# sashakolpakov/graphem-rapids

Hardware: AMD Instinct MI355X
Metric: layout iterations/s (higher is better)
Workload: dtype f32; 1 GPU; rr1m; graph=rr, n_vertices=1000000, n_edges=4000000, n_components=3, n_neighbors=10, sample_size=256, sampler=device, knn=auto, knn_distance=exact, parallelism=rows/1, reference_identical=False

## Files before the change

### graphem-rapids_amd/csrc/api.hip

```cpp
#include "common.h"
#include "engine.h"
#include "qcell_core.h"

#include "torch_randperm.h"

#include <algorithm>
#include <chrono>
#include <condition_variable>
#include <mutex>
#include <new>
#include <thread>
#include <stdlib.h>
#include <string.h>

static thread_local std::string g_create_error;
void gh_set_create_error(const std::string &msg) { g_create_error = msg; }

gh_scope::gh_scope(gh_engine *h_, const char *name, hipStream_t on) : h(h_), stream(on ? on : h_->stream) {
    if (!h->timing) return;
    for (size_t i = 0; i < h->timers.size(); ++i)
        if (h->timers[i].name == name) slot = (int)i;
    if (slot < 0) {
        h->timers.emplace_back();
        h->timers.back().name = name;
// ... 74 lines not shown
    sw.no_presetup = getenv("GRAPHEM_HIP_NO_PRESETUP") != nullptr;
    sw.reorder = getenv("GRAPHEM_HIP_REORDER");
    if (const char *e = getenv("GRAPHEM_HIP_TAU_SEPARATE")) sw.tau_separate = atoi(e) != 0;
    sw.stamps = getenv("GRAPHEM_HIP_STAMPS") != nullptr;
    return sw;
}

static gh_status allocate_and_upload(gh_engine *h, const gh_graph_plan &g, const create_switches &sw) {
    const int64_t n = h->n, E = h->E;
    const int D = h->D;
    const bool hashed = h->part.edge_rule == GH_EDGES_HASHED;
    const size_t nLD = (size_t)n * h->LD, S = (size_t)h->S;
    gh_status st;
#define GH_A(p, count, zero) GH_TRY_ST(gh_alloc(h, h->p, (count), (zero)))
    GH_A(d_edges, (size_t)E * 2, false);
    GH_A(d_rowptr, (size_t)h->rows + 1, false);
    GH_A(d_adj, (size_t)h->adj_len, false);
    GH_A(d_first_edge, (size_t)h->rows + 1, true);
    GH_A(d_mid, (size_t)h->own_count * h->LD, true);
    GH_A(d_Fs, (size_t)h->rows * h->LD, true);
    const bool scan_path = gh_knn_scan_path(h);
    GH_A(d_gmin, (size_t)gh_gmin_floats(h), true);
    GH_A(d_sub_uv, (size_t)h->thr_M1 * 2, false);
    if (hashed) GH_A(d_own_eids, g.own_eids.size() + 1, true);
    if (h->nlong) {
        GH_A(d_long_rows, g.long_rows.size(), false);
        GH_A(d_long_ownptr, g.long_ownptr.size(), false);
        GH_A(d_long_ownadj, g.long_ownadj.size() + 1, true);
        GH_A(d_long_eptr, g.long_eptr.size(), false);
        GH_A(d_long_erow, g.long_erow.size() + 1, false);
        GH_A(d_long_terms, (size_t)h->long_entries * D, false);
        GH_A(d_own_long, g.own_long.size(), false);
    }
    GH_A(d_vblock, g.vblock.size(), false);
    GH_A(d_pos, (size_t)h->pos_rows * h->LD, true);
    GH_A(d_new_buf, (size_t)h->rows * h->LD, true);
    h->d_new = h->d_new_buf.p;
    GH_A(d_tmpF, nLD, true);
    GH_A(d_tmpF2, nLD, true);
    GH_A(d_io, (size_t)n * D, false);
    GH_A(d_acc, nLD, true);
    GH_A(d_tflag, (size_t)n, true);
    GH_A(d_touched, 4 * S * (size_t)h->k, false);
    GH_A(d_tcount, 1, true);
    GH_A(d_sampled, S, true);
    GH_A(d_q, S * (size_t)(h->LD + 4), true);
// ... 244 lines not shown
    }
    if (gh_grid_path(h)) {
        GH_TRY_ST(gh_knn_prepare(h));
        GH_TRY_ST(gh_launch_spring_mid(h));
        GH_TRY_ST(gh_grid_search(h));
        return gh_knn_finish(h, true, fuse_intersect);
    }
    if (gh_ivf_path(h)) {
        GH_TRY_ST(gh_knn_prepare(h));
        GH_TRY_ST(gh_launch_spring_mid(h));
        GH_TRY_ST(gh_ivf_search(h));
        return gh_knn_finish(h, true, fuse_intersect);
    }
    if (h->fused_scan && gh_knn_scan_path(h)) {
        GH_TRY_ST(gh_knn_prepare(h));
        if (!h->tau_embedded) GH_TRY_ST(gh_knn_thresholds(h));
        GH_TRY_ST(gh_launch_spring_scan(h));
        return gh_knn_finish(h, false, fuse_intersect);
    }
    GH_TRY_ST(gh_launch_spring_mid(h));
    return gh_knn_local(h, fuse_intersect);
}

static gh_status step_merge(gh_engine *h, const uint64_t *gathered, int world) {
    GH_TRY_ST(gh_knn_merge(h, gathered, world));
    if (!h->intersect_done) GH_TRY_ST(gh_launch_intersect(h));
    GH_TRY_ST(gh_launch_integrate(h));
    return GH_OK;
}

static gh_status step_finish(gh_engine *h, const gh_ids *next) {
    const bool presetup = next && h->rows == h->n && h->layout != GH_LAYOUT_GATHERED && gh_knn_scan_path(h) &&
                          (h->fused_scan || gh_grid_path(h) || gh_ivf_path(h)) && h->S > 0 && h->k > 0 && !h->opt_no_presetup;
    GH_TRY_ST(gh_launch_normalise(h, true, presetup ? next : nullptr));
    h->iter += 1;
    return GH_OK;
}

template <class Src, class Before>
static gh_status run_iterations(gh_engine *h, int32_t iters, bool draws_own, Src src_of_row, Before before_row) {
    const gh_ids own = gh_own_ids(h);
    auto loop = [&]() -> gh_status {
        for (int32_t t = 0; t < iters; ++t) {
            GH_TRY_ST(before_row(t));
            h->sample = src_of_row(t);
            GH_TRY_ST(step_begin(h, true));
            GH_TRY_ST(step_merge(h, h->d_partial.p, 1));
            const gh_ids next = t + 1 < iters ? src_of_row(t + 1) : own;
            GH_TRY_ST(step_finish(h, t + 1 < iters || draws_own ? &next : nullptr));
        }
        return GH_OK;
    };
    const gh_status st = loop();
    h->sample = gh_ids{GH_IDS_GIVEN, h->d_sampled.p};
    return st;
}
static gh_status nothing_before(int32_t) { return GH_OK; }

extern "C" gh_status gh_step(gh_handle h, const int32_t *sampled) {
    GH_TRY_ST(check_handle(h));
    if (h->f64) return gh_f64_step(h, sampled);
    GH_TRY_ST(check_whole(h, "gh_step"));
    GH_TRY_ST(check_k(h));
    gh_ids src;
    GH_TRY_ST(caller_ids(h, sampled, &src));
    return run_iterations(h, 1, sampled == nullptr, [&](int32_t) { return src; }, nothing_before);
}

static gh_status ensure_stream_ids(gh_engine *h, size_t words) {
    if (words <= h->stream_ids_cap) return GH_OK;
    if (h->d_stream_ids.p) { GH_HIP(hipStreamSynchronize(h->stream)); h->d_stream_ids.reset(); h->stream_ids_cap = 0; }
    GH_TRY_ST(gh_alloc(h, h->d_stream_ids, words, false));
// ... 571 lines not shown
```

### graphem-rapids_amd/csrc/engine.h

```cpp
#pragma once
#include <hip/hip_runtime.h>
#include <stdint.h>
#include <memory>
#include <string>
#include <vector>

#include "../../include/graphem_hip.h"
#include "host_util.h"

#define GH_CAND_CAP 16384
#define GH_SEL_BUF 4096
#define GH_SEL_CHUNK 2048
#define GH_CNT_STRIDE 32
#define GH_POS_PAD_ROWS 1024
inline int gh_fix_blocks(int LD) { return LD <= 16 ? 2 * LD : 0; }
#define GH_SCAN_MIN_EDGES 16384

struct gh_timer_slot {
    std::string name;
    double total_ms = 0.0;
    int64_t launches = 0;
    std::vector<std::pair<hipEvent_t, hipEvent_t>> pending;
};

// ... 83 lines not shown
    float *d_new = nullptr;
    gh_dev<float> d_tmpF;
    gh_dev<float> d_tmpF2;
    gh_dev<float> d_io;

    gh_dev<double> d_acc;
    gh_dev<int32_t> d_tflag;
    gh_dev<int32_t> d_touched;
    gh_dev<int32_t> d_tcount;

    gh_dev<int32_t> d_sampled;
    gh_ids sample{};
    gh_dev<int32_t> d_stream_ids;
    size_t stream_ids_cap = 0;
    gh_ring ring;
    double sampler_stats[4] = {0, 0, 0, 0};
    bool new0_ready = false;
    bool intersect_done = false;
    bool stats_reduced = false;
    struct {
        bool valid = false;
        gh_ids src{};
        uint64_t iter = 0;
    } lookahead;
    bool last_step_own_ids = false;
    bool tcount_reset_pending = false;
    gh_dev<float> d_iscratch;
    gh_dev<float> d_q;
    gh_dev<float> d_qscan;
    gh_dev<uint16_t> d_qA;
    gh_dev<int32_t> d_order;
    std::vector<int32_t> order_host;
    gh_dev<unsigned char> d_gbuf;
    int64_t g_slot = 0, g_chunk = 0;
    int g_world = 0, g_rank = 0;
    int layout = GH_LAYOUT_NONE;
    gh_dev<float> d_rows_packed;
    bool packed_exchange = false;
    bool rows_early = false;
    gh_dev<float> d_rows_all;
    gh_dev<float> d_rows_pk;
    gh_dev<double> d_stats_all;
    int64_t stats_block = 0;
    int64_t patch_cap = 0;
    gh_dev<int32_t> d_qexact;
    gh_dev<uint64_t> d_cand;
    gh_dev<int32_t> d_cnt;
// ... 41 lines not shown
#define GH_STAMP_EXTRA 8192
    gh_dev<unsigned long long> d_stamps;
    bool timing = false;
    std::vector<gh_timer_slot> timers;

    std::unique_ptr<gh_ivf, gh_part_delete> ivf;
    std::unique_ptr<gh_f64, gh_part_delete> f64;
    std::unique_ptr<gh_comm, gh_part_delete> comm;
};

template <class T> gh_status gh_alloc(gh_engine *h, gh_dev<T> &buf, size_t count, bool zero) {
    if (count == 0) count = 1;
    if (!buf.alloc(count * sizeof(T))) {
        h->err = std::string("hipMalloc failed: ") + hipGetErrorString(hipGetLastError());
        return GH_ERR_NOMEM;
    }
    if (zero) GH_HIP(hipMemsetAsync(buf.p, 0, count * sizeof(T), h->stream));
    return GH_OK;
}

inline gh_ids gh_own_ids(const gh_engine *h) { return gh_ids{h->S >= h->E ? GH_IDS_ARANGE : GH_IDS_SAMPLER, h->d_sampled.p}; }
inline void gh_set_lookahead(gh_engine *h, const gh_ids *next) {
    h->lookahead.valid = next != nullptr;
    if (next) { h->lookahead.src = *next; h->lookahead.iter = h->iter + 1; }
}

struct gh_scope {
    gh_engine *h;
    int slot = -1;
    hipEvent_t a = nullptr, b = nullptr;
    hipStream_t stream = nullptr;
    gh_scope(gh_engine *h_, const char *name, hipStream_t on = nullptr );
    ~gh_scope();
};

struct gh_graph_plan {
    const int32_t *edges = nullptr;
    std::vector<int32_t> internal;
    std::vector<int32_t> rowptr, adj;
    std::vector<int32_t> first_edge, own_eids, vblock;
    std::vector<int32_t> long_rows, long_ownptr, long_ownadj, long_eptr, long_erow;
    std::vector<uint8_t> own_long;
    std::vector<int32_t> sub_uv;
};
void gh_plan_graph(gh_engine *h, const int32_t *edges, bool partitioned, int reorder, gh_graph_plan *g);
void gh_auto_knn_method(gh_engine *h);
void gh_plan_threshold_subset(const gh_engine *h, gh_graph_plan *g);
// ... 27 lines not shown
gh_status gh_knn_points_device(hipStream_t stream, const float *d_q, int64_t nq, const float *d_ref, int64_t nref,
                               int D, int K, uint64_t *d_keys, std::string *err);
gh_status gh_cdist_alloc(gh_engine *h);
gh_status gh_knn_merge_cdist(gh_engine *h, const uint64_t *gathered, int world);
gh_status gh_knn_finish_cdist(gh_engine *h, bool all_rows, bool fuse_intersect);
bool gh_grid_path(const gh_engine *h);
gh_status gh_grid_alloc(gh_engine *h);
gh_status gh_grid_search(gh_engine *h);
bool gh_ivf_path(const gh_engine *h);
gh_status gh_ivf_alloc(gh_engine *h);
gh_status gh_ivf_search(gh_engine *h);
gh_status gh_radial_topk_device(gh_engine *h, int K, uint64_t *d_part, int nparts, int32_t *d_ids);
int gh_fused_mfma_kb(const gh_engine *h);
bool gh_fused_uses_mfma(const gh_engine *h);
int gh_fused_tile(const gh_engine *h);
bool gh_fused_cells_ok(const gh_engine *h);
void gh_choose_scan_filter(gh_engine *h);
gh_status gh_launch_spring_scan(gh_engine *h);
gh_status gh_knn_merge(gh_engine *h, const uint64_t *gathered, int world);
gh_status gh_launch_intersect(gh_engine *h);
gh_status gh_launch_inter_cleanup(gh_engine *h);
gh_status gh_launch_spring_mid(gh_engine *h);
gh_status gh_launch_mid_only(gh_engine *h);
gh_status gh_launch_integrate(gh_engine *h);
gh_status gh_launch_spring_only(gh_engine *h, float *d_F);
gh_status gh_launch_inter_to_dense(gh_engine *h, float *d_F);
gh_status gh_launch_integrate_given(gh_engine *h, const float *d_Fs, const float *d_Fi);
gh_status gh_launch_normalise(gh_engine *h, bool with_cleanup, const gh_ids *next = nullptr, bool gathered = false,
                              const double *stats_all = nullptr);
gh_status gh_launch_unpack_rows(gh_engine *h);
struct gh_long_args;
gh_long_args gh_make_long_args(const gh_engine *h, bool coop_mid = false);
gh_status gh_launch_spring_long(gh_engine *h, float *outF, int64_t f_row0);
inline int32_t *gh_patch_count(gh_engine *h) { return reinterpret_cast<int32_t *>(h->d_stats + (size_t)(2 + 2 * gh_fix_blocks(h->LD)) * h->LD); }
inline float *gh_patch_records(gh_engine *h) { return reinterpret_cast<float *>(gh_patch_count(h) + 4); }
gh_status gh_launch_new0(gh_engine *h);
gh_status gh_launch_pack_rows(gh_engine *h, hipStream_t stream);
gh_status gh_launch_patch_rows(gh_engine *h);
gh_status gh_launch_pad(gh_engine *h, const float *d_src_nD, float *d_dst_nLD);
gh_status gh_launch_unpad(gh_engine *h, const float *d_src_nLD, float *d_dst_nD);
gh_status gh_launch_sample(gh_engine *h);
gh_status gh_launch_arange(gh_engine *h);
gh_status gh_ensure_sample(gh_engine *h);
```

### graphem-rapids_amd/csrc/forces.hip

```cpp
#include "common.h"
#include "engine.h"
#include "intersect_core.h"
#include "setup_core.h"

namespace {

template <int D, int LD, bool WRITE_MID, bool LONG>
__global__ __launch_bounds__(256) void spring_kernel(
    const float *__restrict__ pos, const int32_t *__restrict__ rowptr, const int32_t *__restrict__ adj,
    const int32_t *__restrict__ first_edge, int64_t edge_lo, int64_t row_lo, int64_t rows, float L_min,
    float neg_k, float *__restrict__ outF, int64_t f_row0, float *__restrict__ mid, gh_long_args la) {
    const int64_t i = blockIdx.x * (int64_t)blockDim.x + threadIdx.x;
    if (i >= rows) return;
    const int64_t x = row_lo + i;
    float px[LD], F[LD];
    gh_load_row<LD>(pos, x, px);
    int64_t mid_row0 = 0;
    if (WRITE_MID) mid_row0 = first_edge[i] - edge_lo;
    if constexpr (LONG)
        spring_row<D, LD, WRITE_MID>(pos, adj, rowptr[i], rowptr[i + 1], x, px, L_min, neg_k, F, mid, mid_row0, la, (int)i,
                                     outF + (i + f_row0) * LD);
    else
        spring_pull<D, LD, WRITE_MID>(pos, adj, rowptr[i], rowptr[i + 1], x, px, L_min, neg_k, F, mid, mid_row0);
    gh_store_row<LD>(outF, i + f_row0, F);
// ... 194 lines not shown
}

__global__ __launch_bounds__(256) void stats_reduce_kernel(const double *__restrict__ blockstats, int nblocks, int LD,
                                                          double *__restrict__ stats) {
    const int c = blockIdx.x;
    double s = 0.0;
    for (int b = threadIdx.x; b < nblocks; b += blockDim.x) s += blockstats[(int64_t)c * nblocks + b];
    __shared__ double red[4];
    const double a = gh_wave_sum(s);
    if ((threadIdx.x & 63) == 0) red[threadIdx.x >> 6] = a;
    __syncthreads();
    if (threadIdx.x == 0) stats[c] = ((red[0] + red[1]) + red[2]) + red[3];
}

template <int LD>
__global__ __launch_bounds__(256) void stats_fix_kernel(const double *__restrict__ blockstats, int nblocks,
                                                       const float *__restrict__ pos, const float *__restrict__ Fs,
                                                       const double *__restrict__ acc,
                                                       const int32_t *__restrict__ touched,
                                                       const int32_t *__restrict__ tcount, int64_t row_lo,
                                                       int64_t rows, float *__restrict__ out_new,
                                                       double *__restrict__ stats, int skip_reduce,
                                                       int32_t *__restrict__ patch_count = nullptr ,
                                                       float *__restrict__ patch_rows = nullptr, int patch_cap = 0) {
    __shared__ double red[4][2 * LD];
    const int lane = threadIdx.x & 63, w = threadIdx.x >> 6;
    if (!skip_reduce) {
        const int c = blockIdx.x;
        double s = 0.0;
        double s4[4] = {0.0, 0.0, 0.0, 0.0};
        const double *col = blockstats + (int64_t)c * nblocks;
        int b = threadIdx.x;
        for (; b + 3 * (int)blockDim.x < nblocks; b += 4 * blockDim.x) {
#pragma unroll
            for (int u = 0; u < 4; ++u) s4[u] += col[b + u * blockDim.x];
        }
        for (int u = 0; b < nblocks; b += blockDim.x, ++u) s4[u] += col[b];
        s = (s4[0] + s4[1]) + (s4[2] + s4[3]);
        const double a = gh_wave_sum(s);
        if (lane == 0) red[w][0] = a;
        __syncthreads();
        if (threadIdx.x == 0) stats[c] = ((red[0][0] + red[1][0]) + red[2][0]) + red[3][0];
        __syncthreads();
    }
    double dx[LD], dxx[LD];
#pragma unroll
    for (int d = 0; d < LD; ++d) { dx[d] = 0.0; dxx[d] = 0.0; }
    const int nt = *tcount;
    for (int t = blockIdx.x * blockDim.x + threadIdx.x; t < nt; t += gridDim.x * blockDim.x) {
        const int64_t x = touched[t];
        const int64_t i = x - row_lo;
        if (i < 0 || i >= rows) continue;
        float p[LD], f[LD], nw[LD];
        gh_load_row<LD>(pos, x, p);
        gh_load_row<LD>(Fs, i, f);
#pragma unroll
        for (int d = 0; d < LD; ++d) {
            const float n0 = p[d] + f[d];
            const float tot = f[d] + (float)acc[x * LD + d];
            nw[d] = p[d] + tot;
            dx[d] += (double)nw[d] - (double)n0;
            dxx[d] += (double)nw[d] * (double)nw[d] - (double)n0 * (double)n0;
        }
        if (!patch_count) gh_store_row<LD>(out_new, i, nw);
        else gh_patch_append<LD>(patch_count, patch_rows, patch_cap, x, nw);
    }
#pragma unroll
    for (int d = 0; d < LD; ++d) {
        const double a = gh_wave_sum(dx[d]), b = gh_wave_sum(dxx[d]);
        if (lane == 0) { red[w][d] = a; red[w][LD + d] = b; }
    }
    __syncthreads();
// ... 10 lines not shown
        const int64_t x = touched[t / LD];
        const int d = (int)(t % LD);
        acc[x * LD + d] = 0.0;
        if (d == 0) tflag[x] = 0;
    }
}

struct gh_norm_src {
    const float *rows;
    int64_t chunk;
    int64_t block;
    int RS;
    int64_t out_lo, out_rows;
    const double *stats;
    int world;
    int64_t stats_block;
    __device__ const float *row(int64_t j) const {
        const float *p = rows;
        for (; j >= chunk; j -= chunk) p += block;
        return p + j * RS;
    }
};

template <int LDT>
__global__ __launch_bounds__(256) void normalise_kernel(gh_norm_src src, int D, int LD, int64_t n, float *__restrict__ pos,
                                                       double *__restrict__ acc ,
                                                       int32_t *__restrict__ tflag,
                                                       const int32_t *__restrict__ touched,
                                                       const int32_t *__restrict__ tcount, int nfix, int g_norm,
                                                       int n_setup, gh_setup_args sa, int32_t *__restrict__ qexact,
                                                       unsigned long long *__restrict__ stamps ,
                                                       float *__restrict__ packed = nullptr ) {
    if (stamps && (blockIdx.x >= GH_STAMP_EXTRA)) stamps = nullptr;
    if (stamps) stamps += (int64_t)blockIdx.x * 8;
#define GH_STAMP(k) do { if (stamps && threadIdx.x == 0) stamps[k] = wall_clock64(); } while (0)
    GH_STAMP(0);
    __shared__ __align__(16) unsigned char setup_lds[GH_SETUP_LDS_BYTES];
    const bool setup_block = (int)blockIdx.x < n_setup;
    const int nb = (int)blockIdx.x - n_setup;
    if (acc && !setup_block)
        gh_clear_touched(acc, tflag, touched, tcount, LD, nb * (int64_t)blockDim.x + threadIdx.x, (int64_t)g_norm * blockDim.x);
    constexpr int LDS_ = LDT > 0 ? LDT : 4;
    constexpr bool early_fetch = LDT > 0 && LDT <= 8;
    gh_setup_rows<LDS_> srows;
    auto raw_row = [=](int64_t v, float (&row)[LDS_]) {
        const float *p = src.row(v);
        if (src.RS == LD) {
            gh_load_row<LDS_>(p, 0, row);
        } else {
#pragma unroll
            for (int d = 0; d < LDS_; ++d) row[d] = d < D ? p[d] : 0.0f;
        }
    };
    if constexpr (early_fetch)
        if (setup_block && sa.tiles > 0) gh_setup_fetch<LDS_>(sa, (int)blockIdx.x, raw_row, srows);
    extern __shared__ float ms[];
    double *srow = reinterpret_cast<double *>(ms + 2 * LD);
    const int R = 2 + 2 * nfix;
    double *tot = srow + R * LD;
    for (int r = 0; r < src.world; ++r) {
        const double *st = src.stats + (int64_t)r * src.stats_block;
        for (int t = threadIdx.x; t < R * LD; t += blockDim.x) srow[t] = st[t];
        __syncthreads();
        for (int d = threadIdx.x; d < LD; d += blockDim.x) {
            double sum = srow[d], sq = srow[LD + d];
#pragma unroll 8
            for (int b = 0; b < nfix; ++b) {
                sum += srow[(2 + 2 * b) * LD + d];
                sq += srow[(3 + 2 * b) * LD + d];
            }
            sum = (r > 0 ? tot[d] : 0.0) + sum;
            sq = (r > 0 ? tot[LD + d] : 0.0) + sq;
            if (r + 1 < src.world) {
                tot[d] = sum;
                tot[LD + d] = sq;
                continue;
            }
            float mean = 0.0f, sd = 1.0f;
            if (d < D) {
                const double m = sum / (double)n;
                double var = (sq - sum * m) / (double)(n - 1);
                if (var < 0.0) var = 0.0;
                mean = (float)m;
                sd = (float)sqrt(var) + 1e-6f;
            }
            ms[d] = mean;
            ms[LD + d] = sd;
        }
        __syncthreads();
    }
    GH_STAMP(1);
    if (stamps && threadIdx.x == 0) stamps[6] = setup_block ? 1 : 2;
    if (setup_block) {
        const int64_t t = (int64_t)blockIdx.x * blockDim.x + threadIdx.x;
        if (t == 0) qexact[0] = 0;
        auto getp = [=](int64_t v, int d) { return (src.row(v)[d] - ms[d]) / ms[LD + d]; };
        if constexpr (LDT > 0) {
            if (sa.tiles > 0) {
                auto norm = [=](float x, int d) { return (x - ms[d]) / ms[LD + d]; };
                if constexpr (!early_fetch) gh_setup_fetch<LDS_>(sa, (int)blockIdx.x, raw_row, srows);
                gh_setup_finish<LDS_>(sa, (int)blockIdx.x, raw_row, norm, srows, setup_lds, stamps);
            } else {
                gh_setup_item(sa, t, getp);
            }
        } else {
            gh_setup_item(sa, t, getp);
        }
        GH_STAMP(3);
        return;
    }
    const int64_t step = (int64_t)g_norm * blockDim.x;
    const float *in = src.rows;
    for (int64_t j0 = 0; j0 < src.out_rows; j0 += src.chunk, in += src.block) {
        const int64_t total4 = min(src.chunk, src.out_rows - j0) * LD / 4;
        float4 *dst = reinterpret_cast<float4 *>(pos + (src.out_lo + j0) * LD);
        auto norm4 = [&](int64_t t, const float4 &v) {
            const int d0 = (int)((t * 4) % LD);
            float4 o;
            o.x = d0 + 0 < D ? (v.x - ms[d0 + 0]) / ms[LD + d0 + 0] : 0.0f;
            o.y = d0 + 1 < D ? (v.y - ms[d0 + 1]) / ms[LD + d0 + 1] : 0.0f;
            o.z = d0 + 2 < D ? (v.z - ms[d0 + 2]) / ms[LD + d0 + 2] : 0.0f;
            o.w = d0 + 3 < D ? (v.w - ms[d0 + 3]) / ms[LD + d0 + 3] : 0.0f;
            dst[t] = o;
            if (packed) {
// ... 253 lines not shown
    if (M == 0) return GH_OK;
    gh_scope t(h, "mid_gather");
    mid_gather_kernel<<<dim3(grid_for(M * h->LD, 256)), dim3(256), 0, h->stream>>>(
        h->d_pos.p, h->d_edges.p, h->part.edge_lo, h->d_own_eids.p, M, h->D, h->LD, h->d_mid.p);
    GH_LAUNCH_CHECK();
    return GH_OK;
}

}

gh_status gh_launch_spring_mid(gh_engine *h) {
    const bool fused = h->fused_mid && gh_dim_templated(h->D);
    if (h->rows > 0) {
        gh_scope t(h, fused ? "spring_mid" : "spring");
        gh_status st = fused ? launch_spring<true>(h, h->d_Fs.p, 0) : launch_spring<false>(h, h->d_Fs.p, 0);
        if (st) return st;
    }
    if (!fused) return launch_mid_gather(h);
    return GH_OK;
}

gh_status gh_launch_mid_only(gh_engine *h) { return launch_mid_gather(h); }

gh_status gh_launch_integrate(gh_engine *h) {
    if (h->new0_ready && h->rows > 0) {
        h->new0_ready = false;
        gh_scope t(h, "stats_fix");
        const struct reset_flag { gh_engine *e; ~reset_flag() { e->stats_reduced = false; } } reset{h};
        if (!gh_dispatch_stride(h->LD, [&](auto ld) {
                stats_fix_kernel<ld()><<<dim3(gh_fix_blocks(ld())), dim3(256), 0, h->stream>>>(
                    h->d_blockstats.p, h->n_vblocks, h->d_pos.p, h->d_Fs.p, h->d_acc.p, h->d_touched.p, h->d_tcount.p, h->part.row_lo,
                    h->rows, h->d_new, h->d_stats, h->stats_reduced ? 1 : 0,
                    h->layout == GH_LAYOUT_OVERLAP ? gh_patch_count(h) + (h->iter & 1) : nullptr,
                    h->layout == GH_LAYOUT_OVERLAP ? gh_patch_records(h) : nullptr, (int)h->patch_cap);
            })) {
            h->err = "stats_fix: the fused step left its sums for a row stride other than 4, 8 or 16";
            return GH_ERR_RUNTIME;
        }
        GH_LAUNCH_CHECK();
        return GH_OK;
    }
    h->new0_ready = false;
    GH_HIP(hipMemsetAsync(h->d_stats + 2 * h->LD, 0, sizeof(double) * 2 * gh_fix_blocks(h->LD) * h->LD, h->stream));
    if (h->rows == 0) {
        GH_HIP(hipMemsetAsync(h->d_stats, 0, sizeof(double) * 2 * h->LD, h->stream));
        return GH_OK;
    }
    const unsigned grid = grid_for(h->rows, 256);
    int32_t *pc = h->layout == GH_LAYOUT_OVERLAP ? gh_patch_count(h) + (h->iter & 1) : nullptr;
    float *pr = h->layout == GH_LAYOUT_OVERLAP ? gh_patch_records(h) : nullptr;
    const int pcap = (int)h->patch_cap;
    float *wide_out = h->d_new;
    {
        gh_scope t(h, "integrate");
        if (!gh_dispatch_stride(h->LD, [&](auto ld) {
                integrate_kernel<ld()><<<dim3(grid), dim3(256), 0, h->stream>>>(h->d_pos.p, h->d_Fs.p, h->part.row_lo, h->rows, h->d_acc.p,
                                                                               h->d_tflag.p, h->d_new, h->d_blockstats.p, pc, pr, pcap);
            }))
            integrate_generic_kernel<<<dim3(grid_for(h->rows * h->LD, 256)), dim3(256), 0, h->stream>>>(
                h->d_pos.p, h->d_Fs.p, h->LD, h->part.row_lo, h->rows, h->d_acc.p, h->d_tflag.p, wide_out);
        GH_LAUNCH_CHECK();
    }
// ... 43 lines not shown

gh_status gh_launch_inter_cleanup(gh_engine *h) {
    const int64_t maxT = 4 * h->S * h->k * h->LD;
    if (maxT == 0) return GH_OK;
    gh_scope t(h, "inter_cleanup");
    inter_cleanup_kernel<<<dim3(grid_for(maxT, 256)), dim3(256), 0, h->stream>>>(h->d_acc.p, h->d_tflag.p, h->d_touched.p,
                                                                                 h->d_tcount.p, h->LD);
    reset_counter_kernel<<<dim3(1), dim3(1), 0, h->stream>>>(h->d_tcount.p);
    GH_LAUNCH_CHECK();
    return GH_OK;
}

gh_status gh_launch_integrate_given(gh_engine *h, const float *d_Fs, const float *d_Fi) {
    GH_HIP(hipMemsetAsync(h->d_stats, 0, sizeof(double) * (2 + 2 * gh_fix_blocks(h->LD)) * h->LD, h->stream));
    const int64_t total = h->n * h->LD;
    integrate_given_kernel<<<dim3(grid_for(total, 256)), dim3(256), 0, h->stream>>>(h->d_pos.p, d_Fs, d_Fi, total,
                                                                                    h->d_new);
    column_stats_kernel<<<dim3(h->D), dim3(256), 0, h->stream>>>(h->d_new, h->n, h->D, h->LD, h->d_stats);
    GH_LAUNCH_CHECK();
    return GH_OK;
}

gh_status gh_launch_normalise(gh_engine *h, bool with_cleanup, const gh_ids *next, bool gathered, const double *stats_all) {
    gh_set_lookahead(h, nullptr);
    const int R = 2 + 2 * gh_fix_blocks(h->LD);
    gh_norm_src src{h->d_new, std::max<int64_t>(h->rows, 1), 0, h->LD, h->part.row_lo, h->rows, h->d_stats, 1, 0};
    if (stats_all) {
        src.stats = stats_all;
        src.world = h->g_world;
        src.stats_block = (int64_t)R * h->LD;
    }
    if (gathered) {
        const bool overlap = h->layout == GH_LAYOUT_OVERLAP;
        src.RS = overlap && h->d_rows_pk.p ? h->D : h->LD;
        src.rows = overlap ? (h->d_rows_pk.p ? h->d_rows_pk.p : h->d_rows_all.p) : reinterpret_cast<const float *>(h->d_gbuf.p);
        src.chunk = std::min(h->g_chunk, h->n);
        src.block = overlap ? h->g_chunk * src.RS : h->g_slot / (int64_t)sizeof(float);
        src.out_lo = 0;
        src.out_rows = h->n;
        src.stats = overlap ? h->d_stats_all.p : reinterpret_cast<const double *>(h->d_gbuf.p + h->g_chunk * h->LD * (int64_t)sizeof(float));
        src.world = h->g_world;
        src.stats_block = overlap ? h->stats_block : h->g_slot / (int64_t)sizeof(double);
        if (!(h->fused_scan && gh_knn_scan_path(h) && h->S > 0 && h->k > 0 && !h->opt_no_presetup)) next = nullptr;
    }
    if (src.out_rows == 0) return with_cleanup ? gh_launch_inter_cleanup(h) : GH_OK;
    gh_scope t(h, gathered ? "normalise_gathered" : stats_all ? "normalise_own" : "normalise");
    unsigned grid = grid_for(src.out_rows * h->LD / 4, 1024);
    if (grid > 2048) grid = 2048;
    gh_setup_args sa{};
    unsigned extra = 0;
    if (next) {
        sa = gh_make_setup_args(h, *next, h->iter + 1);
        extra = gh_setup_blocks(sa);
    }
    const size_t smem = sizeof(float) * 2 * h->LD + sizeof(double) * (size_t)(R + (src.world > 1 ? 2 : 0)) * h->LD;
    float *packed = stats_all && h->packed_exchange ? h->d_rows_packed.p + (size_t)h->g_rank * h->g_chunk * h->D : nullptr;
    const int ldt = stats_all ? 0 : h->LD;
    const auto normalise = [&](auto ld) {
        normalise_kernel<ld()><<<dim3(grid + extra), dim3(256), smem, h->stream>>>(
            src, h->D, h->LD, h->n, h->d_pos.p, with_cleanup ? h->d_acc.p : nullptr, h->d_tflag.p, h->d_touched.p, h->d_tcount.p,
            gh_fix_blocks(h->LD), (int)grid, (int)extra, sa, h->d_qexact.p,
            h->d_stamps.p ? h->d_stamps.p + (int64_t)std::max(h->n_vblocks, 1) * 8 : nullptr, packed);
    };
    if (!gh_dispatch_stride(ldt, normalise)) {
        if (sa.tiles > 0) { h->err = "KNN set-up tiles need a row stride of 4, 8 or 16"; return GH_ERR_RUNTIME; }
        normalise(gh_int<0>{});
    }
    GH_LAUNCH_CHECK();
    gh_set_lookahead(h, next);
    return GH_OK;
}

__global__ __launch_bounds__(256) void unpack_rows_kernel(const float *__restrict__ packed, int64_t n, int D, int LD, int64_t own_lo,
                                                         int64_t own_hi, float *__restrict__ pos) {
    const int64_t t = blockIdx.x * (int64_t)256 + threadIdx.x;
    if (t >= n * LD) return;
    const int64_t row = t / LD;
    const int d = (int)(t % LD);
    if (row >= own_lo && row < own_hi) return;
    pos[t] = d < D ? packed[row * D + d] : 0.0f;
}
gh_status gh_launch_unpack_rows(gh_engine *h) {
    if (!h->packed_exchange) return GH_OK;
    gh_scope t(h, "unpack_rows");
    unpack_rows_kernel<<<dim3(grid_for(h->n * h->LD, 256)), dim3(256), 0, h->stream>>>(h->d_rows_packed.p, h->n, h->D, h->LD, h->part.row_lo,
// ... 111 lines not shown
```

### graphem-rapids_amd/csrc/knn.hip

```cpp
#include "common.h"
#include "engine.h"
#include "scan_core.h"
#include "setup_core.h"
#include "tau_core.h"
#include "intersect_core.h"
#include "select_core.h"

#include <math.h>
#include <type_traits>
#include <stdlib.h>

namespace {


__global__ __launch_bounds__(256) void knn_setup_kernel(const float *__restrict__ pos, gh_setup_args a,
                                                       int32_t *__restrict__ tcount, int32_t *__restrict__ qexact) {
    __shared__ __align__(16) unsigned char lds[GH_SETUP_LDS_BYTES];
    if (blockIdx.x == 0 && threadIdx.x == 0) { *tcount = 0; qexact[0] = 0; }
    const int LD = a.LD;
    auto getp = [=](int64_t v, int d) { return pos[v * LD + d]; };
    if (a.tiles > 0) gh_setup_block_any(a, (int)blockIdx.x, getp, lds);
    else gh_setup_item(a, blockIdx.x * (int64_t)blockDim.x + threadIdx.x, getp);
}

// ... 439 lines not shown
    return GH_OK;
}

}

static int64_t own_edges(const gh_engine *h) { return h->own_count; }

bool gh_knn_scan_path(const gh_engine *h) {
    const int64_t Mtot = own_edges(h);
    return Mtot >= GH_SCAN_MIN_EDGES && h->LD <= 16 && h->D >= 2 && h->Ksel <= GH_EXTRACT_MAX_K && h->S <= 0x7FFFFFFF;
}

void gh_choose_threshold_subset(gh_engine *h) {
    const int64_t Mtot = own_edges(h);
    const bool scan = gh_knn_scan_path(h) && !gh_grid_path(h) && !gh_ivf_path(h);
    h->thr_stride = scan ? subset_stride(Mtot, h->Ksel, h->S, gh_fused_tile(h), gh_fused_uses_mfma(h)) : 1;
    h->thr_M1 = scan ? (Mtot + h->thr_stride - 1) / h->thr_stride : 0;
}

gh_setup_args gh_make_setup_args(const gh_engine *h, gh_ids src, uint64_t iter) {
    const int tiles = (int)((h->thr_M1 + GH_THR_TILE - 1) / GH_THR_TILE);
    return gh_setup_args{h->d_edges.p, src.ids, src.mode, h->E, h->prm.seed, iter, h->S, h->D, h->LD, h->d_q.p, h->d_cnt.p,
                         h->d_ovf.p, h->part.edge_lo, h->d_own_eids.p, reinterpret_cast<const int2 *>(h->d_sub_uv.p), h->thr_M1, h->thr_stride, h->d_gmin.p,
                         (int64_t)tiles * GH_THR_GROUPS, tiles, h->tau_embedded ? h->d_tau_flag.p : nullptr};
}

unsigned gh_setup_blocks(const gh_setup_args &a) {
    return a.tiles > 0 ? (unsigned)a.tiles : (unsigned)((a.S + 255) / 256);
}
int64_t gh_gmin_floats(const gh_engine *h) {
    const gh_setup_args a = gh_make_setup_args(h, gh_ids{GH_IDS_GIVEN, nullptr}, 0);
    if (gh_ivf_path(h)) return h->S * 256 + 4;
    if (a.tiles == 0) return 4;
    return h->S * a.Gpad + 4;
}

gh_status gh_knn_prepare(gh_engine *h) {
    const gh_ids src = h->sample;
    h->sample.mode = GH_IDS_GIVEN;
    const bool done = h->lookahead.valid && h->lookahead.iter == h->iter && h->lookahead.src.mode == src.mode &&
                      h->lookahead.src.ids == src.ids;
    gh_set_lookahead(h, nullptr);
    h->tcount_reset_pending = done;
    if (done) return GH_OK;
    const gh_setup_args a = gh_make_setup_args(h, src, h->iter);
    gh_scope t(h, "knn_setup");
    knn_setup_kernel<<<dim3(gh_setup_blocks(a)), dim3(256), 0, h->stream>>>(h->d_pos.p, a, h->d_tcount.p, h->d_qexact.p);
// ... 178 lines not shown
```

### graphem-rapids_amd/csrc/setup_core.h

```cpp
#pragma once
#include "common.h"
#include "engine.h"
#include "scan_core.h"

struct gh_setup_args {
    const int32_t *edges;
    int32_t *sampled;
    int mode;
    int64_t E;
    uint64_t seed, iter;
    int64_t S;
    int D, LD;
    float *qt;
    int32_t *cnt, *ovf;
    int64_t e_lo;
    const int32_t *own_eids;
    const int2 *sub_uv;
    int64_t M1, stride;
    float *gmin;
    int64_t Gpad;
    int tiles;
    unsigned *tau_flag;
};

#define GH_THR_TILE 128
#define GH_THR_GSIZE 64
#define GH_THR_GROUPS (GH_THR_TILE / GH_THR_GSIZE)

template <class P >
__device__ __forceinline__ void gh_setup_item(const gh_setup_args &a, int64_t t, P getp) {
    if (t == 0 && a.tau_flag) *a.tau_flag = 0;
    if (t >= a.S) return;
    int32_t e32;
    if (a.mode == 1) { e32 = gh_sample_id(a.E, a.seed, a.iter, t); a.sampled[t] = e32; }
    else if (a.mode == 2) { e32 = (int32_t)t; a.sampled[t] = e32; }
    else e32 = a.sampled[t];
    const int QS = gh_qs(a.D, a.LD);
    const int64_t e = e32;
    const int64_t u = a.edges[2 * e], v = a.edges[2 * e + 1];
    for (int d = 0; d < QS; ++d) a.qt[t * QS + d] = d < a.D ? (getp(u, d) + getp(v, d)) / 2.0f : 0.0f;
    a.qt[t * QS + gh_qtau(a.D, a.LD)] = INFINITY;
    a.cnt[t * GH_CNT_STRIDE] = 0;
    a.ovf[t] = 0;
}

template <int CTRL>
__device__ __forceinline__ uint32_t gh_dpp_u32(uint32_t v) {
    return (uint32_t)__builtin_amdgcn_update_dpp((int)v, (int)v, CTRL, 0xF, 0xF, false);
}
__device__ __forceinline__ uint32_t gh_row_min_u32(uint32_t v) {
    v = min(v, gh_dpp_u32<0xB1>(v));
    v = min(v, gh_dpp_u32<0x4E>(v));
    v = min(v, gh_dpp_u32<0x141>(v));
    v = min(v, gh_dpp_u32<0x140>(v));
    return v;
}

#define GH_SETUP_LDS_BYTES (GH_THR_TILE * 16 * 4)
template <int LD>
struct gh_setup_rows {
    float qa[LD], qb[LD], ma[LD], mb[LD];
    int32_t e32;
};
template <int LD, class RAW >
__device__ __forceinline__ void gh_setup_fetch(const gh_setup_args &a, int blk, RAW raw, gh_setup_rows<LD> &st) {
    const int t = threadIdx.x;
    __builtin_amdgcn_s_setprio(3);
    if (blk == 0 && t == 0 && a.tau_flag) *a.tau_flag = 0;
    st.e32 = 0;
#pragma unroll
    for (int d = 0; d < LD; ++d) { st.qa[d] = 0.0f; st.qb[d] = 0.0f; st.ma[d] = 0.0f; st.mb[d] = 0.0f; }
    if (t < a.S) {
        if (a.mode == 1) st.e32 = gh_sample_id(a.E, a.seed, a.iter, t);
        else if (a.mode == 2) st.e32 = (int32_t)t;
        else st.e32 = a.sampled[t];
        const int2 uv = reinterpret_cast<const int2 *>(a.edges)[st.e32];
        raw(uv.x, st.qa);
        raw(uv.y, st.qb);
    }
    if (t < GH_THR_TILE) {
        const int64_t j = (int64_t)blk * GH_THR_TILE + t;
        if (j < a.M1) {
            const int2 uv = a.sub_uv[j];
            raw(uv.x, st.ma);
            raw(uv.y, st.mb);
        }
    }
}

template <int LD, class RAW, class NORM >
__device__ __forceinline__ void gh_setup_finish(const gh_setup_args &a, int blk, RAW raw, NORM norm, const gh_setup_rows<LD> &st,
                                                unsigned char *lds, unsigned long long *stamps = nullptr ) {
    gh_f2 *rsh = reinterpret_cast<gh_f2 *>(lds);
    const int t = threadIdx.x;
    auto query = [&](int64_t s, int32_t &e32, float (&q)[LD]) {
        if (a.mode == 1) e32 = gh_sample_id(a.E, a.seed, a.iter, s);
        else if (a.mode == 2) e32 = (int32_t)s;
        else e32 = a.sampled[s];
        const int2 uv = reinterpret_cast<const int2 *>(a.edges)[e32];
        float ra[LD], rb[LD];
        raw(uv.x, ra);
        raw(uv.y, rb);
#pragma unroll
        for (int d = 0; d < LD; ++d) q[d] = d < a.D ? (norm(ra[d], d) + norm(rb[d], d)) / 2.0f : 0.0f;
    };
    float q[LD];
    int32_t e32 = st.e32;
#pragma unroll
    for (int d = 0; d < LD; ++d) q[d] = d < a.D ? (norm(st.qa[d], d) + norm(st.qb[d], d)) / 2.0f : 0.0f;
    if (t < GH_THR_TILE) {
        const int64_t j = (int64_t)blk * GH_THR_TILE + t;
        float m[LD];
#pragma unroll
        for (int d = 0; d < LD; ++d) m[d] = 0.0f;
        if (j < a.M1) {
#pragma unroll
            for (int d = 0; d < LD; ++d)
                if (d < a.D) m[d] = (norm(st.ma[d], d) + norm(st.mb[d], d)) / 2.0f;
        } else {
            m[0] = INFINITY;
        }
        float *slot = reinterpret_cast<float *>(rsh + (t >> 1) * LD) + (t & 1);
#pragma unroll
        for (int d = 0; d < LD; ++d) slot[2 * d] = m[d];
    }
// ... 36 lines not shown
            }
            mn[gg] = best;
        }
        static_assert(GH_THR_GROUPS == 2 || GH_THR_GROUPS % 4 == 0, "vector stores of the group minima");
        if constexpr (GH_THR_GROUPS == 2) {
            *reinterpret_cast<uint2 *>(dst) = make_uint2(mn[0], mn[1]);
        } else {
#pragma unroll
            for (int g4 = 0; g4 < GH_THR_GROUPS; g4 += 4)
                *reinterpret_cast<uint4 *>(dst + g4) = make_uint4(mn[g4], mn[g4 + 1], mn[g4 + 2], mn[g4 + 3]);
        }
    }
}

template <int LD, class P>
__device__ __forceinline__ void gh_setup_block(const gh_setup_args &a, int blk, P getp, unsigned char *lds,
                                               unsigned long long *stamps = nullptr ) {
    auto raw = [&](int64_t v, float (&row)[LD]) {
#pragma unroll
        for (int d = 0; d < LD; ++d) row[d] = d < a.D ? getp(v, d) : 0.0f;
    };
    auto norm = [](float x, int) { return x; };
    gh_setup_rows<LD> st;
    gh_setup_fetch<LD>(a, blk, raw, st);
    gh_setup_finish<LD>(a, blk, raw, norm, st, lds, stamps);
}

template <class P>
__device__ __forceinline__ void gh_setup_block_any(const gh_setup_args &a, int blk, P getp, unsigned char *lds,
                                                   unsigned long long *stamps = nullptr) {
    if (a.LD == 4) gh_setup_block<4>(a, blk, getp, lds, stamps);
    else if (a.LD == 8) gh_setup_block<8>(a, blk, getp, lds, stamps);
    else gh_setup_block<16>(a, blk, getp, lds, stamps);
}
```

Baseline: 6496 iterations/s.

## Stage next-iteration KNN setup endpoint rows during stats_fix kernel

The stats_fix launch gains extra blocks that gather the next iteration's sampled edge endpoint rows (new position computed from pos, Fs and acc, or taken from new0) into a staging buffer. The normalise kernel's KNN setup tiles can then read those contiguous rows instead of doing random edge and position lookups. This moves scattered gather latency into a kernel that was lightly occupied and removes repeated per-tile random reads. It adds a buffer, a lookahead validity flag and a second template instantiation, and it depends on the staged rows matching what normalise would have computed.

```diff
diff --git a/graphem-rapids_amd/csrc/api.hip b/graphem-rapids_amd/csrc/api.hip
--- a/graphem-rapids_amd/csrc/api.hip
+++ b/graphem-rapids_amd/csrc/api.hip
@@ -120,6 +120,7 @@
     const bool scan_path = gh_knn_scan_path(h);
     GH_A(d_gmin, (size_t)gh_gmin_floats(h), true);
     GH_A(d_sub_uv, (size_t)h->thr_M1 * 2, false);
+    if (h->thr_M1 > 0 && h->rows == n) GH_A(d_setup_rows, 2 * S * h->LD, true);
     if (hashed) GH_A(d_own_eids, g.own_eids.size() + 1, true);
     if (h->nlong) {
         GH_A(d_long_rows, g.long_rows.size(), false);
@@ -410,17 +411,20 @@
     return gh_knn_local(h, fuse_intersect);
 }
 
-static gh_status step_merge(gh_engine *h, const uint64_t *gathered, int world) {
+static gh_status step_merge(gh_engine *h, const uint64_t *gathered, int world, const gh_ids *next = nullptr) {
     GH_TRY_ST(gh_knn_merge(h, gathered, world));
     if (!h->intersect_done) GH_TRY_ST(gh_launch_intersect(h));
-    GH_TRY_ST(gh_launch_integrate(h));
-    return GH_OK;
-}
-
-static gh_status step_finish(gh_engine *h, const gh_ids *next) {
+    GH_TRY_ST(gh_launch_integrate(h, next));
+    return GH_OK;
+}
+
+static const gh_ids *presetup_ids(const gh_engine *h, const gh_ids *next) {
     const bool presetup = next && h->rows == h->n && h->layout != GH_LAYOUT_GATHERED && gh_knn_scan_path(h) &&
                           (h->fused_scan || gh_grid_path(h) || gh_ivf_path(h)) && h->S > 0 && h->k > 0 && !h->opt_no_presetup;
-    GH_TRY_ST(gh_launch_normalise(h, true, presetup ? next : nullptr));
+    return presetup ? next : nullptr;
+}
+static gh_status step_finish(gh_engine *h, const gh_ids *next) {
+    GH_TRY_ST(gh_launch_normalise(h, true, presetup_ids(h, next)));
     h->iter += 1;
     return GH_OK;
 }
@@ -433,9 +437,10 @@
             GH_TRY_ST(before_row(t));
             h->sample = src_of_row(t);
             GH_TRY_ST(step_begin(h, true));
-            GH_TRY_ST(step_merge(h, h->d_partial.p, 1));
             const gh_ids next = t + 1 < iters ? src_of_row(t + 1) : own;
-            GH_TRY_ST(step_finish(h, t + 1 < iters || draws_own ? &next : nullptr));
+            const gh_ids *next_ids = t + 1 < iters || draws_own ? &next : nullptr;
+            GH_TRY_ST(step_merge(h, h->d_partial.p, 1, presetup_ids(h, next_ids)));
+            GH_TRY_ST(step_finish(h, next_ids));
         }
         return GH_OK;
     };
diff --git a/graphem-rapids_amd/csrc/engine.h b/graphem-rapids_amd/csrc/engine.h
--- a/graphem-rapids_amd/csrc/engine.h
+++ b/graphem-rapids_amd/csrc/engine.h
@@ -129,7 +129,9 @@
         bool valid = false;
         gh_ids src{};
         uint64_t iter = 0;
+        bool rows = false;
     } lookahead;
+    gh_dev<float> d_setup_rows;
     bool last_step_own_ids = false;
     bool tcount_reset_pending = false;
     gh_dev<float> d_iscratch;
@@ -217,7 +219,18 @@
 inline gh_ids gh_own_ids(const gh_engine *h) { return gh_ids{h->S >= h->E ? GH_IDS_ARANGE : GH_IDS_SAMPLER, h->d_sampled.p}; }
 inline void gh_set_lookahead(gh_engine *h, const gh_ids *next) {
     h->lookahead.valid = next != nullptr;
+    h->lookahead.rows = false;
     if (next) { h->lookahead.src = *next; h->lookahead.iter = h->iter + 1; }
+}
+inline void gh_set_lookahead_rows(gh_engine *h, const gh_ids &next) {
+    h->lookahead.valid = false;
+    h->lookahead.rows = true;
+    h->lookahead.src = next;
+    h->lookahead.iter = h->iter + 1;
+}
+inline bool gh_lookahead_rows_for(const gh_engine *h, const gh_ids *next) {
+    return next && h->lookahead.rows && h->lookahead.iter == h->iter + 1 && h->lookahead.src.mode == next->mode &&
+           h->lookahead.src.ids == next->ids;
 }
 
 struct gh_scope {
@@ -291,7 +304,7 @@
 gh_status gh_launch_inter_cleanup(gh_engine *h);
 gh_status gh_launch_spring_mid(gh_engine *h);
 gh_status gh_launch_mid_only(gh_engine *h);
-gh_status gh_launch_integrate(gh_engine *h);
+gh_status gh_launch_integrate(gh_engine *h, const gh_ids *next = nullptr);
 gh_status gh_launch_spring_only(gh_engine *h, float *d_F);
 gh_status gh_launch_inter_to_dense(gh_engine *h, float *d_F);
 gh_status gh_launch_integrate_given(gh_engine *h, const float *d_Fs, const float *d_Fi);
diff --git a/graphem-rapids_amd/csrc/forces.hip b/graphem-rapids_amd/csrc/forces.hip
--- a/graphem-rapids_amd/csrc/forces.hip
+++ b/graphem-rapids_amd/csrc/forces.hip
@@ -240,7 +240,14 @@
                                                        int64_t rows, float *__restrict__ out_new,
                                                        double *__restrict__ stats, int skip_reduce,
                                                        int32_t *__restrict__ patch_count = nullptr ,
-                                                       float *__restrict__ patch_rows = nullptr, int patch_cap = 0) {
+                                                       float *__restrict__ patch_rows = nullptr, int patch_cap = 0,
+                                                       gh_setup_args sa = gh_setup_args{} ,
+                                                       const int32_t *__restrict__ tflag = nullptr, float *__restrict__ setup_rows = nullptr) {
+    constexpr int NFIX = 2 * LD;
+    if ((int)blockIdx.x >= NFIX) {
+        gh_setup_gather<LD>(sa, gh_gather_src{pos, Fs, out_new, acc, tflag, setup_rows}, (int)blockIdx.x - NFIX);
+        return;
+    }
     __shared__ double red[4][2 * LD];
     const int lane = threadIdx.x & 63, w = threadIdx.x >> 6;
     if (!skip_reduce) {
@@ -265,7 +272,7 @@
 #pragma unroll
     for (int d = 0; d < LD; ++d) { dx[d] = 0.0; dxx[d] = 0.0; }
     const int nt = *tcount;
-    for (int t = blockIdx.x * blockDim.x + threadIdx.x; t < nt; t += gridDim.x * blockDim.x) {
+    for (int t = blockIdx.x * blockDim.x + threadIdx.x; t < nt; t += NFIX * blockDim.x) {
         const int64_t x = touched[t];
         const int64_t i = x - row_lo;
         if (i < 0 || i >= rows) continue;
@@ -322,7 +329,7 @@
     }
 };
 
-template <int LDT>
+template <int LDT, bool STAGED>
 __global__ __launch_bounds__(256) void normalise_kernel(gh_norm_src src, int D, int LD, int64_t n, float *__restrict__ pos,
                                                        double *__restrict__ acc ,
                                                        int32_t *__restrict__ tflag,
@@ -353,7 +360,7 @@
         }
     };
     if constexpr (early_fetch)
-        if (setup_block && sa.tiles > 0) gh_setup_fetch<LDS_>(sa, (int)blockIdx.x, raw_row, srows);
+        if (setup_block && sa.tiles > 0) gh_setup_fetch<LDS_, STAGED>(sa, (int)blockIdx.x, raw_row, srows);
     extern __shared__ float ms[];
     double *srow = reinterpret_cast<double *>(ms + 2 * LD);
     const int R = 2 + 2 * nfix;
@@ -398,8 +405,8 @@
         if constexpr (LDT > 0) {
             if (sa.tiles > 0) {
                 auto norm = [=](float x, int d) { return (x - ms[d]) / ms[LD + d]; };
-                if constexpr (!early_fetch) gh_setup_fetch<LDS_>(sa, (int)blockIdx.x, raw_row, srows);
-                gh_setup_finish<LDS_>(sa, (int)blockIdx.x, raw_row, norm, srows, setup_lds, stamps);
+                if constexpr (!early_fetch) gh_setup_fetch<LDS_, STAGED>(sa, (int)blockIdx.x, raw_row, srows);
+                gh_setup_finish<LDS_, STAGED>(sa, (int)blockIdx.x, raw_row, norm, srows, setup_lds, stamps);
             } else {
                 gh_setup_item(sa, t, getp);
             }
@@ -699,22 +706,31 @@
 
 gh_status gh_launch_mid_only(gh_engine *h) { return launch_mid_gather(h); }
 
-gh_status gh_launch_integrate(gh_engine *h) {
+gh_status gh_launch_integrate(gh_engine *h, const gh_ids *next) {
+    h->lookahead.rows = false;
     if (h->new0_ready && h->rows > 0) {
         h->new0_ready = false;
         gh_scope t(h, "stats_fix");
         const struct reset_flag { gh_engine *e; ~reset_flag() { e->stats_reduced = false; } } reset{h};
+        gh_setup_args sa{};
+        unsigned gather = 0;
+        if (next && h->d_setup_rows.p && h->rows == h->n && h->part.row_lo == 0 && h->layout == GH_LAYOUT_NONE) {
+            sa = gh_make_setup_args(h, *next, h->iter + 1);
+            if (sa.tiles > 0) gather = gh_gather_blocks(sa.S);
+        }
         if (!gh_dispatch_stride(h->LD, [&](auto ld) {
-                stats_fix_kernel<ld()><<<dim3(gh_fix_blocks(ld())), dim3(256), 0, h->stream>>>(
+                stats_fix_kernel<ld()><<<dim3(gh_fix_blocks(ld()) + gather), dim3(256), 0, h->stream>>>(
                     h->d_blockstats.p, h->n_vblocks, h->d_pos.p, h->d_Fs.p, h->d_acc.p, h->d_touched.p, h->d_tcount.p, h->part.row_lo,
                     h->rows, h->d_new, h->d_stats, h->stats_reduced ? 1 : 0,
                     h->layout == GH_LAYOUT_OVERLAP ? gh_patch_count(h) + (h->iter & 1) : nullptr,
-                    h->layout == GH_LAYOUT_OVERLAP ? gh_patch_records(h) : nullptr, (int)h->patch_cap);
+                    h->layout == GH_LAYOUT_OVERLAP ? gh_patch_records(h) : nullptr, (int)h->patch_cap, sa, h->d_tflag.p,
+                    h->d_setup_rows.p);
             })) {
             h->err = "stats_fix: the fused step left its sums for a row stride other than 4, 8 or 16";
             return GH_ERR_RUNTIME;
         }
         GH_LAUNCH_CHECK();
+        if (gather) gh_set_lookahead_rows(h, *next);
         return GH_OK;
     }
     h->new0_ready = false;
@@ -804,6 +820,7 @@
 }
 
 gh_status gh_launch_normalise(gh_engine *h, bool with_cleanup, const gh_ids *next, bool gathered, const double *stats_all) {
+    const bool staged = !gathered && !stats_all && gh_lookahead_rows_for(h, next);
     gh_set_lookahead(h, nullptr);
     const int R = 2 + 2 * gh_fix_blocks(h->LD);
     gh_norm_src src{h->d_new, std::max<int64_t>(h->rows, 1), 0, h->LD, h->part.row_lo, h->rows, h->d_stats, 1, 0};
@@ -834,15 +851,22 @@
     if (next) {
         sa = gh_make_setup_args(h, *next, h->iter + 1);
         extra = gh_setup_blocks(sa);
+        if (staged && sa.tiles > 0) sa.rows = h->d_setup_rows.p;
     }
     const size_t smem = sizeof(float) * 2 * h->LD + sizeof(double) * (size_t)(R + (src.world > 1 ? 2 : 0)) * h->LD;
     float *packed = stats_all && h->packed_exchange ? h->d_rows_packed.p + (size_t)h->g_rank * h->g_chunk * h->D : nullptr;
     const int ldt = stats_all ? 0 : h->LD;
     const auto normalise = [&](auto ld) {
-        normalise_kernel<ld()><<<dim3(grid + extra), dim3(256), smem, h->stream>>>(
-            src, h->D, h->LD, h->n, h->d_pos.p, with_cleanup ? h->d_acc.p : nullptr, h->d_tflag.p, h->d_touched.p, h->d_tcount.p,
-            gh_fix_blocks(h->LD), (int)grid, (int)extra, sa, h->d_qexact.p,
-            h->d_stamps.p ? h->d_stamps.p + (int64_t)std::max(h->n_vblocks, 1) * 8 : nullptr, packed);
+        const auto launch = [&](auto kernel) {
+            kernel<<<dim3(grid + extra), dim3(256), smem, h->stream>>>(
+                src, h->D, h->LD, h->n, h->d_pos.p, with_cleanup ? h->d_acc.p : nullptr, h->d_tflag.p, h->d_touched.p, h->d_tcount.p,
+                gh_fix_blocks(h->LD), (int)grid, (int)extra, sa, h->d_qexact.p,
+                h->d_stamps.p ? h->d_stamps.p + (int64_t)std::max(h->n_vblocks, 1) * 8 : nullptr, packed);
+        };
+        if constexpr (ld() > 0) {
+            if (sa.rows) return launch(normalise_kernel<ld(), true>);
+        }
+        launch(normalise_kernel<ld(), false>);
     };
     if (!gh_dispatch_stride(ldt, normalise)) {
         if (sa.tiles > 0) { h->err = "KNN set-up tiles need a row stride of 4, 8 or 16"; return GH_ERR_RUNTIME; }
diff --git a/graphem-rapids_amd/csrc/knn.hip b/graphem-rapids_amd/csrc/knn.hip
--- a/graphem-rapids_amd/csrc/knn.hip
+++ b/graphem-rapids_amd/csrc/knn.hip
@@ -485,7 +485,8 @@
     const int tiles = (int)((h->thr_M1 + GH_THR_TILE - 1) / GH_THR_TILE);
     return gh_setup_args{h->d_edges.p, src.ids, src.mode, h->E, h->prm.seed, iter, h->S, h->D, h->LD, h->d_q.p, h->d_cnt.p,
                          h->d_ovf.p, h->part.edge_lo, h->d_own_eids.p, reinterpret_cast<const int2 *>(h->d_sub_uv.p), h->thr_M1, h->thr_stride, h->d_gmin.p,
-                         (int64_t)tiles * GH_THR_GROUPS, tiles, h->tau_embedded ? h->d_tau_flag.p : nullptr};
+                         (int64_t)tiles * GH_THR_GROUPS, tiles, h->tau_embedded ? h->d_tau_flag.p : nullptr,
+                         nullptr };
 }
 
 unsigned gh_setup_blocks(const gh_setup_args &a) {
diff --git a/graphem-rapids_amd/csrc/setup_core.h b/graphem-rapids_amd/csrc/setup_core.h
--- a/graphem-rapids_amd/csrc/setup_core.h
+++ b/graphem-rapids_amd/csrc/setup_core.h
@@ -21,6 +21,7 @@
     int64_t Gpad;
     int tiles;
     unsigned *tau_flag;
+    const float *rows;
 };
 
 #define GH_THR_TILE 128
@@ -62,7 +63,12 @@
     float qa[LD], qb[LD], ma[LD], mb[LD];
     int32_t e32;
 };
-template <int LD, class RAW >
+__device__ __forceinline__ int32_t gh_setup_id(const gh_setup_args &a, int64_t s) {
+    if (a.mode == 1) return gh_sample_id(a.E, a.seed, a.iter, s);
+    if (a.mode == 2) return (int32_t)s;
+    return a.sampled[s];
+}
+template <int LD, bool STAGED , class RAW >
 __device__ __forceinline__ void gh_setup_fetch(const gh_setup_args &a, int blk, RAW raw, gh_setup_rows<LD> &st) {
     const int t = threadIdx.x;
     __builtin_amdgcn_s_setprio(3);
@@ -71,12 +77,16 @@
 #pragma unroll
     for (int d = 0; d < LD; ++d) { st.qa[d] = 0.0f; st.qb[d] = 0.0f; st.ma[d] = 0.0f; st.mb[d] = 0.0f; }
     if (t < a.S) {
-        if (a.mode == 1) st.e32 = gh_sample_id(a.E, a.seed, a.iter, t);
-        else if (a.mode == 2) st.e32 = (int32_t)t;
-        else st.e32 = a.sampled[t];
-        const int2 uv = reinterpret_cast<const int2 *>(a.edges)[st.e32];
-        raw(uv.x, st.qa);
-        raw(uv.y, st.qb);
+        if constexpr (STAGED) {
+            if (blk == 0) st.e32 = gh_setup_id(a, t);
+            gh_load_row<LD>(a.rows, 2 * (int64_t)t, st.qa);
+            gh_load_row<LD>(a.rows, 2 * (int64_t)t + 1, st.qb);
+        } else {
+            st.e32 = gh_setup_id(a, t);
+            const int2 uv = reinterpret_cast<const int2 *>(a.edges)[st.e32];
+            raw(uv.x, st.qa);
+            raw(uv.y, st.qb);
+        }
     }
     if (t < GH_THR_TILE) {
         const int64_t j = (int64_t)blk * GH_THR_TILE + t;
@@ -88,19 +98,51 @@
     }
 }
 
-template <int LD, class RAW, class NORM >
+struct gh_gather_src {
+    const float *pos, *Fs, *new0;
+    const double *acc;
+    const int32_t *tflag;
+    float *rows;
+};
+inline unsigned gh_gather_blocks(int64_t S) { return (unsigned)((2 * S + 255) / 256); }
+template <int LD>
+__device__ __forceinline__ void gh_setup_gather(const gh_setup_args &a, const gh_gather_src &g, int blk) {
+    const int64_t r = (int64_t)blk * 256 + threadIdx.x;
+    if (r >= 2 * a.S) return;
+    const int64_t x = a.edges[2 * (int64_t)gh_setup_id(a, r >> 1) + (r & 1)];
+    float row[LD];
+    if (g.tflag[x] == 0) {
+        gh_load_row<LD>(g.new0, x, row);
+    } else {
+        float p[LD], f[LD];
+        gh_load_row<LD>(g.pos, x, p);
+        gh_load_row<LD>(g.Fs, x, f);
+#pragma unroll
+        for (int d = 0; d < LD; ++d) {
+            const float tot = f[d] + (float)g.acc[x * LD + d];
+            row[d] = p[d] + tot;
+        }
+    }
+    gh_store_row<LD>(g.rows, r, row);
+}
+
+template <int LD, bool STAGED, class RAW, class NORM >
 __device__ __forceinline__ void gh_setup_finish(const gh_setup_args &a, int blk, RAW raw, NORM norm, const gh_setup_rows<LD> &st,
                                                 unsigned char *lds, unsigned long long *stamps = nullptr ) {
     gh_f2 *rsh = reinterpret_cast<gh_f2 *>(lds);
     const int t = threadIdx.x;
     auto query = [&](int64_t s, int32_t &e32, float (&q)[LD]) {
-        if (a.mode == 1) e32 = gh_sample_id(a.E, a.seed, a.iter, s);
-        else if (a.mode == 2) e32 = (int32_t)s;
-        else e32 = a.sampled[s];
-        const int2 uv = reinterpret_cast<const int2 *>(a.edges)[e32];
         float ra[LD], rb[LD];
-        raw(uv.x, ra);
-        raw(uv.y, rb);
+        if constexpr (STAGED) {
+            if (blk == 0) e32 = gh_setup_id(a, s);
+            gh_load_row<LD>(a.rows, 2 * s, ra);
+            gh_load_row<LD>(a.rows, 2 * s + 1, rb);
+        } else {
+            e32 = gh_setup_id(a, s);
+            const int2 uv = reinterpret_cast<const int2 *>(a.edges)[e32];
+            raw(uv.x, ra);
+            raw(uv.y, rb);
+        }
 #pragma unroll
         for (int d = 0; d < LD; ++d) q[d] = d < a.D ? (norm(ra[d], d) + norm(rb[d], d)) / 2.0f : 0.0f;
     };
@@ -183,8 +225,8 @@
     };
     auto norm = [](float x, int) { return x; };
     gh_setup_rows<LD> st;
-    gh_setup_fetch<LD>(a, blk, raw, st);
-    gh_setup_finish<LD>(a, blk, raw, norm, st, lds, stamps);
+    gh_setup_fetch<LD, false>(a, blk, raw, st);
+    gh_setup_finish<LD, false>(a, blk, raw, norm, st, lds, stamps);
 }
 
 template <class P>
```

Result: faster. 6611 iterations/s (median of 6 runs) (+1.8%).
